# 10XGenomics/scan-rs

Hardware: NVIDIA B200
Metric: normalize+PCA cells/s, 1.3Mx33.5k, k=10 (higher is better)
Workload: dtype f64

## Files before the change

### scan_rs_b200/csrc/gather.cu

```cuda
#include <cub/cub.cuh>

#include <algorithm>
#include <numeric>

#include "common.cuh"
#include "map.cuh"

#define FULLMASK 0xffffffffu
#define GA_THREADS 1024
#define GA_STAGE_STRIDE 176u
#define GA_NONE 0xFFFFFFFFu
#define GA_TILE 20u

#define GA_ST_KEYS 16u
#define GA_ST_XS 48u
#define GA_ST_L1 112u

template <int MODE, int TAIL>
__global__ void __launch_bounds__(GA_THREADS, 1)
k_gather(const uint2 *__restrict__ ent, const GUnit *__restrict__ units, const u32 *__restrict__ item_first, u32 n_units, u32 n_items,
         u32 *__restrict__ tickets, u32 ticket_base, u32 rows, u64 n_cells, MapDev mp, const double *__restrict__ B, u32 ldb, u32 col0, u32 wt, u32 w,
         const u32 *__restrict__ slot_gene, double *__restrict__ out, u32 ldo, long long *__restrict__ cycles) {
    __shared__ u32 s_item;
    __shared__ long long s_t0;
    if (cycles && threadIdx.x == 0) s_t0 = clock64();
    extern __shared__ __align__(16) unsigned char smem_raw[];
    double *XA = reinterpret_cast<double *>(smem_raw);
    double *XB = XA + (size_t)(rows + 1) * 16;
    double *par = XB + (TAIL ? (size_t)(rows + 1) * 4 : 0);
    double *par2 = par + rows;
    LogEnt *ltab = reinterpret_cast<LogEnt *>(par2 + rows);
    unsigned char *stage_all = reinterpret_cast<unsigned char *>(ltab + 128);

    const int lane = threadIdx.x & 31, wib = threadIdx.x >> 5, nw = blockDim.x >> 5;
    const int grp = lane >> 3, lig = lane & 7;
    const u32 xa_sa = (u32)__cvta_generic_to_shared(XA) + (u32)lig * 16u;
    const u32 xb_sa = (u32)__cvta_generic_to_shared(XB) + (u32)(lig & 3) * 8u;
    const u32 stage_grp = (u32)__cvta_generic_to_shared(stage_all) + (u32)(wib * 4 + grp) * GA_STAGE_STRIDE;
    const u32 zero_off16 = rows * 8u;
    const u32 cA = 2u * lig, cB = 16u + (lig & 3);
    const bool ok0 = cA < wt && col0 + cA < w, ok1 = cA + 1 < wt && col0 + cA + 1 < w;
    const bool okb = TAIL && cB < wt && col0 + cB < w;
    const u32 wt_even = (wt + 1) & ~1u;
    const bool logchain = mp.kind == 1;
    constexpr bool TS = MODE >= 1, DEFER = MODE == 2;
    double *const oA = out + col0 + cA;
    const long long tdelta = (long long)cB - (long long)cA;
    const u32 ok0m = ok0, ok1m = ok1, okbm = okb;
    const u64 ldo64 = (u64)ldo;

    for (int i = threadIdx.x; i < 128; i += blockDim.x) ltab[i] = sb_log_table[i];

    u32 staged = GA_NONE;
    u32 first_item = GA_NONE;

    for (;;) {
    __syncthreads();
    if (threadIdx.x == 0) s_item = atomicAdd(tickets, 1u) - ticket_base;
    __syncthreads();
    const u32 item = s_item;
    if (item >= n_items) break;
    if (first_item == GA_NONE) first_item = item;
    const u32 u_begin = item_first[item], u_end = min(n_units, item_first[item + 1]);
    for (u32 ui = u_begin; ui < u_end; ui++) {
        const GUnit un = units[ui];
        if (un.panel != staged) {
            __syncthreads();
            constexpr u32 PAIRS = TAIL ? 10 : 8;
            for (u32 i = threadIdx.x; i < (rows + 1) * PAIRS; i += blockDim.x) {
                const u32 r = i / PAIRS, j2 = (i - r * PAIRS) * 2, col = col0 + j2;
                double2 val = make_double2(0.0, 0.0);
                if (r < rows && j2 < wt_even && col < w) {
                    if (MODE == 0) {
                        const u64 cell = (u64)un.panel * rows + r;
                        if (cell < n_cells) {
                            val = *reinterpret_cast<const double2 *>(B + cell * (size_t)ldb + col);
                            if (logchain) {
                                const double l1 = mp.l1[cell];
                                val.x *= l1;
                                val.y *= l1;
                            }
                        }
                    } else {
                        const u32 g = slot_gene[(size_t)un.panel * rows + r];
                        if (g != GA_NONE) {
                            val = *reinterpret_cast<const double2 *>(B + (size_t)g * ldb + col);
                            if (logchain && mp.row) {
                                const double rs = mp.row[g];
                                val.x *= rs;
                                val.y *= rs;
                            }
                        }
                    }
                }
                if (j2 < 16) *reinterpret_cast<double2 *>(XA + (size_t)r * 16 + j2) = val;
                else *reinterpret_cast<double2 *>(XB + (size_t)r * 4 + (j2 - 16)) = val;
            }
            for (u32 r = threadIdx.x; r < rows; r += blockDim.x) {
                double pv = 0.0, pv2 = 0.0;
                if (MODE == 0) {
                    const u64 cell = (u64)un.panel * rows + r;
                    if (cell < n_cells) {
                        pv = mp.col[cell];
                        if (logchain) pv2 = mp.inv_l1[cell];
                    }
                } else if (!logchain) {
                    const u32 g = slot_gene[(size_t)un.panel * rows + r];
                    if (g != GA_NONE) pv = mp.row[g];
                }
                par[r] = pv;
                par2[r] = pv2;
            }
            staged = un.panel;
            __syncthreads();
        }
        u64 span = (un.end - un.begin + nw - 1) / nw;
        span = (span + 31) & ~(u64)31;
        const u64 wb = min(un.end, un.begin + (u64)wib * span), we = min(un.end, wb + span);
        const u64 qspan = span >> 2;
        const u64 gb = min(we, wb + (u64)grp * qspan), ge = min(we, gb + qspan);
        const u32 nchunks = (u32)((min(we, wb + qspan) - wb + 7) >> 3);

        u32 cur = GA_NONE, carry = GA_NONE;
        double curL1 = 0.0;
        double a0 = 0.0, a1 = 0.0, bt = 0.0;

        auto flush = [&]() {
            if (cur == GA_NONE) return;
            if (TS && !DEFER) {
                a0 *= curL1;
                a1 *= curL1;
                bt *= curL1;
            }
            double *o = oA + (u64)cur * ldo64;
            asm volatile("{ .reg .pred p; setp.ne.u32 p, %2, 0; @p red.global.add.f64 [%0], %1; }" ::"l"(o), "d"(a0), "r"(ok0m) : "memory");
            asm volatile("{ .reg .pred p; setp.ne.u32 p, %2, 0; @p red.global.add.f64 [%0 + 8], %1; }" ::"l"(o), "d"(a1), "r"(ok1m) : "memory");
            if (TAIL) asm volatile("{ .reg .pred p; setp.ne.u32 p, %2, 0; @p red.global.add.f64 [%0], %1; }" ::"l"(o + tdelta), "d"(bt), "r"(okbm) : "memory");
            a0 = 0.0;
            a1 = 0.0;
            bt = 0.0;
        };

        uint2 znext = (gb + lig < ge) ? __ldcs(ent + gb + lig) : make_uint2(GA_NONE, 0u);
        for (u32 ch = 0; ch < nchunks; ch++) {
            const uint2 z = znext;
            const u64 kn = gb + (u64)(ch + 1) * 8 + lig;
            znext = (kn < ge) ? __ldcs(ent + kn) : make_uint2(GA_NONE, 0u);
            const bool valid = z.x != GA_NONE;
            const u32 key = z.x & SB_GENE_MASK, local = z.x >> SB_GENE_BITS;
            const bool general = valid && (!logchain || z.y != 1u);
            double x = 0.0;
            if (general) {
                if (MODE == 0) {
                    if (logchain) x = map_log_part(mp.log_base, par[local], z.y, ltab) * par2[local];
                    else x = map_full(mp, z.y, key, par[local], false, ltab);
                } else {
                    const double cp = mp.col[key];
                    if (logchain) x = map_log_part(mp.log_base, cp, z.y, ltab) * mp.inv_l1[key];
                    else x = mp.kind == 2 ? map_binom_dev((double)z.y, cp, par[local]) : map_binom_pearson((double)z.y, cp, par[local]);
                }
            }
            u32 prev = __shfl_up_sync(FULLMASK, key, 1, 8);
            if (lig == 0) prev = carry;
            const bool head = valid && key != prev;
            double l1v = 0.0;
            if (TS && !DEFER && head) l1v = logchain ? mp.l1[key] : 1.0;
            carry = __shfl_sync(FULLMASK, key, 7, 8);
            const u32 myh = (__ballot_sync(FULLMASK, head) >> (8 * grp)) & 0xFFu;
            const u32 myg = (__ballot_sync(FULLMASK, general) >> (8 * grp)) & 0xFFu;
            __syncwarp();
            asm volatile("st.shared.u16 [%0], %1;" ::"r"(stage_grp + (u32)lig * 2u), "h"((unsigned short)(valid ? local * 8u : zero_off16)) : "memory");
            asm volatile("st.shared.u32 [%0], %1;" ::"r"(stage_grp + GA_ST_KEYS + (u32)lig * 4u), "r"(key) : "memory");
            if (general) asm volatile("st.shared.f64 [%0], %1;" ::"r"(stage_grp + GA_ST_XS + (u32)lig * 8u), "d"(x) : "memory");
            if (TS && !DEFER && head) asm volatile("st.shared.f64 [%0], %1;" ::"r"(stage_grp + GA_ST_L1 + (u32)lig * 8u), "d"(l1v) : "memory");
            __syncwarp();
            u32 ov[4];
            asm volatile("ld.shared.v4.u32 {%0, %1, %2, %3}, [%4];" : "=r"(ov[0]), "=r"(ov[1]), "=r"(ov[2]), "=r"(ov[3]) : "r"(stage_grp));
#pragma unroll
            for (int s = 0; s < 8; s += 2) {
                const u32 off0 = (ov[s >> 1] & 0xFFFFu) << 4, off1 = (ov[s >> 1] >> 16) << 4;
                double tl = 0.0;
                if (TAIL) {
                    const u32 toff = (lig < 4 ? off0 : off1) >> 2;
                    asm volatile("ld.shared.f64 %0, [%1];" : "=d"(tl) : "r"(xb_sa + toff));
                }
                double x0, x1, m0 = 1.0, m1 = 1.0;
                asm volatile("{ .reg .pred p; setp.ne.u32 p, %1, 0; @p ld.shared.f64 %0, [%2]; }"
                             : "+d"(m0) : "r"(myg & (1u << s)), "r"(stage_grp + GA_ST_XS + (u32)s * 8u));
                asm volatile("{ .reg .pred p; setp.ne.u32 p, %1, 0; @p ld.shared.f64 %0, [%2]; }"
                             : "+d"(m1) : "r"(myg & (2u << s)), "r"(stage_grp + GA_ST_XS + (u32)(s + 1) * 8u));
                if (myh & (1u << s)) {
                    flush();
                    asm volatile("ld.shared.u32 %0, [%1];" : "=r"(cur) : "r"(stage_grp + GA_ST_KEYS + (u32)s * 4u));
                    if (TS && !DEFER) asm volatile("ld.shared.f64 %0, [%1];" : "=d"(curL1) : "r"(stage_grp + GA_ST_L1 + (u32)s * 8u));
                }
                asm volatile("ld.shared.v2.f64 {%0, %1}, [%2];" : "=d"(x0), "=d"(x1) : "r"(xa_sa + off0));
                a0 = fma(m0, x0, a0);
                a1 = fma(m0, x1, a1);
                if (TAIL && lig < 4) bt = fma(m0, tl, bt);
                if (myh & (2u << s)) {
                    flush();
                    asm volatile("ld.shared.u32 %0, [%1];" : "=r"(cur) : "r"(stage_grp + GA_ST_KEYS + (u32)(s + 1) * 4u));
                    if (TS && !DEFER) asm volatile("ld.shared.f64 %0, [%1];" : "=d"(curL1) : "r"(stage_grp + GA_ST_L1 + (u32)(s + 1) * 8u));
                }
                asm volatile("ld.shared.v2.f64 {%0, %1}, [%2];" : "=d"(x0), "=d"(x1) : "r"(xa_sa + off1));
                a0 = fma(m1, x0, a0);
                a1 = fma(m1, x1, a1);
                if (TAIL && lig >= 4) bt = fma(m1, tl, bt);
            }
        }
        flush();
    }
    }
    if (cycles && threadIdx.x == 0 && first_item != GA_NONE) {
        u32 smid;
        asm volatile("mov.u32 %0, %%smid;" : "=r"(smid));
        cycles[first_item] = clock64() - s_t0;
        cycles[gridDim.x + first_item] = (long long)smid;
    }
}

__global__ void k_t_init(double *__restrict__ out, u64 n, u32 w, u32 ldo, const double *__restrict__ uy, const double *__restrict__ v) {
    const u64 total = n * w;
    for (u64 i = (u64)blockIdx.x * blockDim.x + threadIdx.x; i < total; i += (u64)gridDim.x * blockDim.x) {
        const u64 c = i / w;
        const u32 j = (u32)(i - c * w);
        out[c * ldo + j] = uy ? (v ? v[c] : 1.0) * uy[j] : 0.0;
    }
}

int gather_t_init(sb_ctx *ctx, double *out, u64 n, u32 w, u32 ldo, const double *uy, const double *v) {
    if (n == 0 || w == 0) return SB_OK;
    u64 blocks = std::min<u64>((n * w + 255) / 256, (u64)ctx->sm_count * 16);
    k_t_init<<<(unsigned)blocks, 256, 0, ctx->stream>>>(out, n, w, ldo, uy, v);
    count_launch(ctx);
    return SB_OK;
}

static size_t gather_smem(u32 rows, bool tail) {
    return (size_t)(rows + 1) * (tail ? 20 : 16) * 8 + (size_t)rows * 16 + 128 * sizeof(LogEnt) + (size_t)(GA_THREADS / 32) * 4 * GA_STAGE_STRIDE;
}

int gather_run_tile(sb_ctx *ctx, const GatherLayout &L, int mode, const MapDev &mp, u64 n_cells, const double *B, u32 ldb, u32 w, u32 col0, double *out,
                    u32 ldo, long long *cycles) {
    if (!L.ready) return sb_fail(SB_ERR_UNSUPPORTED, "gather_run: layout not built");
    if (L.nnz == 0 || L.n_units == 0 || w == 0 || col0 >= w) return SB_OK;
    const u32 n_items = L.n_items ? L.n_items : L.grid;
    if (!L.tickets.p) {
        SB_TRY(L.tickets.alloc(1));
        SB_CUDA(cudaMemsetAsync(L.tickets.p, 0, sizeof(u32), ctx->stream));
        L.ticket_base = 0;
    }
    if (L.ticket_base > 0x7F000000u) {
        SB_CUDA(cudaMemsetAsync(L.tickets.p, 0, sizeof(u32), ctx->stream));
        L.ticket_base = 0;
    }
    const u32 wt = std::min(GA_TILE, w - col0);
    const bool tail = wt > 16;
    const size_t smem = gather_smem(L.rows, tail);
    cudaError_t e;
#define GA_LAUNCH(M, T)                                                                                                                        \
    e = cudaFuncSetAttribute(k_gather<M, T>, cudaFuncAttributeMaxDynamicSharedMemorySize, (int)smem);                                          \
    if (e == cudaSuccess)                                                                                                                      \
        k_gather<M, T><<<L.grid, GA_THREADS, smem, ctx->stream>>>(L.ent, L.units.p, L.cta_first.p, L.n_units, n_items, L.tickets.p, L.ticket_base, \
                                                                  L.rows, n_cells, mp, B, ldb, col0, wt, w, L.slot_gene.p, out, ldo, cycles);
    if (mode == 0) {
        if (tail) { GA_LAUNCH(0, 1) } else { GA_LAUNCH(0, 0) }
    } else if (mode == 1) {
        if (tail) { GA_LAUNCH(1, 1) } else { GA_LAUNCH(1, 0) }
    } else {
        if (tail) { GA_LAUNCH(2, 1) } else { GA_LAUNCH(2, 0) }
    }
#undef GA_LAUNCH
    if (e != cudaSuccess) return sb_fail(SB_ERR_CUDA, "gather_run: %zu B of shared memory: %s", smem, cudaGetErrorString(e));
    L.ticket_base += n_items + L.grid;
    count_launch(ctx);
    SB_CUDA(cudaGetLastError());
    return SB_OK;
}

int gather_run(sb_ctx *ctx, const GatherLayout &L, int mode, const MapDev &mp, u64 n_cells, const double *B, u32 ldb, u32 w, double *out, u32 ldo,
               long long *cycles) {
    for (u32 col0 = 0; col0 < w; col0 += GA_TILE) SB_TRY(gather_run_tile(ctx, L, mode, mp, n_cells, B, ldb, w, col0, out, ldo, col0 == 0 ? cycles : nullptr));
    return SB_OK;
}

int gather_build_n(sb_mat *mt, GatherLayout &L, const uint2 *gm, const u64 *gm_base_dev, u64 nnz) {
    sb_ctx *ctx = mt->ctx;
    L.ready = false;
    L.rows = (mt->pc + 1) & ~1u;
    if (L.rows != mt->pc) return sb_fail(SB_ERR_UNSUPPORTED, "gather_build_n: odd panel size");
    L.npanels = mt->np;
    L.ent = gm;
    L.nnz = nnz;
    std::vector<u64> base((size_t)mt->np + 1, 0);
    if (mt->np) SB_CUDA(cudaMemcpyAsync(base.data(), gm_base_dev, base.size() * sizeof(u64), cudaMemcpyDeviceToHost, ctx->stream));
    SB_CUDA(cudaStreamSynchronize(ctx->stream));
    const u32 G = (u32)ctx->sm_count;
    std::vector<GUnit> units;
    std::vector<u32> first;
    gather_units_n(base, nnz, G, units, first);
    L.n_units = (u32)units.size();
    L.grid = G;
    SB_TRY(L.units.alloc(units.size()));
    SB_TRY(L.cta_first.alloc(first.size()));
    if (!units.empty()) SB_CUDA(cudaMemcpyAsync(L.units.p, units.data(), units.size() * sizeof(GUnit), cudaMemcpyHostToDevice, ctx->stream));
    SB_CUDA(cudaMemcpyAsync(L.cta_first.p, first.data(), first.size() * sizeof(u32), cudaMemcpyHostToDevice, ctx->stream));
    SB_CUDA(cudaStreamSynchronize(ctx->stream));
    L.ready = true;
    return SB_OK;
}

__global__ void k_ent_gene_hist(const uint2 *__restrict__ ent, u64 nnz, u32 *__restrict__ hist) {
    for (u64 i = (u64)blockIdx.x * blockDim.x + threadIdx.x; i < nnz; i += (u64)gridDim.x * blockDim.x) atomicAdd(&hist[ent[i].x], 1u);
}

__global__ void k_make_tkeys(const u64 *__restrict__ ptr, const uint2 *__restrict__ ent, u64 nc, u64 c0, const u32 *__restrict__ slot_of_gene,
                             u32 rows, u32 npanels, u32 *__restrict__ keys, u64 *__restrict__ payload) {
    u64 warp = ((u64)blockIdx.x * blockDim.x + threadIdx.x) >> 5;
    u64 nwarps = ((u64)gridDim.x * blockDim.x) >> 5;
    int lane = threadIdx.x & 31;
    for (u64 v = warp; v < nc; v += nwarps) {
        const u64 s = ptr[v], e = ptr[v + 1];
        const u32 blk = (u32)(v / GA_TBLOCK);
        const u32 cell = (u32)(c0 + v);
        for (u64 k = s + lane; k < e; k += 32) {
            const uint2 z = ent[k];
            const u32 slot = slot_of_gene[z.x];
            const u32 p = slot / rows, sl = slot - p * rows;
            keys[k] = blk * npanels + p;
            payload[k] = ((u64)z.y << 32) | (u64)(cell | (sl << SB_GENE_BITS));
        }
    }
}

__global__ void k_unpack_u64(const u64 *__restrict__ payload, uint2 *__restrict__ out, u64 nnz) {
    for (u64 i = (u64)blockIdx.x * blockDim.x + threadIdx.x; i < nnz; i += (u64)gridDim.x * blockDim.x) {
        const u64 p = payload[i];
        out[i] = make_uint2((u32)p, (u32)(p >> 32));
    }
}

__global__ void k_key_first(const u32 *__restrict__ keys, const u64 *__restrict__ payload, u64 nnz, u64 *__restrict__ first,
                            unsigned long long *__restrict__ runs) {
    const int lane = threadIdx.x & 31;
    const u64 total = (nnz + 31) & ~(u64)31;
    for (u64 i = (u64)blockIdx.x * blockDim.x + threadIdx.x; i < total; i += (u64)gridDim.x * blockDim.x) {
        const bool valid = i < nnz;
        const u32 key = valid ? keys[i] : 0xFFFFFFFFu;
        bool head = false;
        if (valid) {
            const bool newkey = i == 0 || keys[i - 1] != key;
            if (newkey) first[key] = i;
            head = newkey || ((u32)payload[i - 1] & SB_GENE_MASK) != ((u32)payload[i] & SB_GENE_MASK);
        }
        const u32 key0 = __shfl_sync(FULLMASK, key, 0);
        const unsigned hm = __ballot_sync(FULLMASK, head);
        if (__all_sync(FULLMASK, !valid || key == key0)) {
            if (lane == 0 && hm) atomicAdd(&runs[key0], (unsigned long long)__popc(hm));
        } else if (head) {
            atomicAdd(&runs[key], 1ull);
        }
    }
}

static inline int ga_grid(u64 items, int threads, sb_ctx *ctx, int per_sm = 16) {
    u64 blocks = (items + threads - 1) / threads, cap = (u64)ctx->sm_count * per_sm;
    return (int)std::max<u64>(1, std::min(blocks, cap));
}

int gather_assign_slots(sb_mat *mt, const uint2 *ent, u64 nnz) {
    sb_ctx *ctx = mt->ctx;
    GatherLayout &L = mt->gt;
    L.ready = false;
    const u32 m = mt->m;
    u32 rows = std::min<u32>(SB_MAX_PANEL_CELLS, (m + 1) & ~1u);
    if (rows < 2) rows = 2;
    L.rows = rows;
    L.npanels = (m + rows - 1) / rows;
    if (L.npanels == 0) L.npanels = 1;
    DevBuf<u32> hist;
    SB_TRY(hist.alloc((size_t)m + 1));
    SB_CUDA(cudaMemsetAsync(hist.p, 0, ((size_t)m + 1) * sizeof(u32), ctx->stream));
    if (nnz) {
        k_ent_gene_hist<<<ga_grid(nnz, 256, ctx), 256, 0, ctx->stream>>>(ent, nnz, hist.p);
        count_launch(ctx);
    }
    std::vector<u32> h((size_t)m + 1);
    SB_CUDA(cudaMemcpyAsync(h.data(), hist.p, h.size() * sizeof(u32), cudaMemcpyDeviceToHost, ctx->stream));
    SB_CUDA(cudaStreamSynchronize(ctx->stream));
    std::vector<u32> order(m);
    std::iota(order.begin(), order.end(), 0u);
    std::stable_sort(order.begin(), order.end(), [&](u32 a, u32 b) { return h[a] > h[b]; });
    std::vector<u32> slot_of(m ? m : 1, 0), slot_gene((size_t)L.npanels * rows, GA_NONE);
    for (u32 r = 0; r < m; r++) {
        slot_of[order[r]] = r;
        slot_gene[r] = order[r];
    }
    SB_TRY(mt->slot_of_gene.alloc(slot_of.size()));
    SB_TRY(L.slot_gene.alloc(slot_gene.size()));
    SB_CUDA(cudaMemcpyAsync(mt->slot_of_gene.p, slot_of.data(), slot_of.size() * sizeof(u32), cudaMemcpyHostToDevice, ctx->stream));
    SB_CUDA(cudaMemcpyAsync(L.slot_gene.p, slot_gene.data(), slot_gene.size() * sizeof(u32), cudaMemcpyHostToDevice, ctx->stream));
    SB_CUDA(cudaStreamSynchronize(ctx->stream));
    return SB_OK;
}

int gather_build_t_range(sb_mat *mt, u64 c0, u64 nc, const u64 *ptr_local, const uint2 *ent, u64 nnz, DevBuf<uint2> &out, std::vector<u64> &seg_len,
                         std::vector<u64> &seg_runs) {
    sb_ctx *ctx = mt->ctx;
    GatherLayout &L = mt->gt;
    const u64 nblk = (nc + GA_TBLOCK - 1) / GA_TBLOCK;
    const u64 nkeys = nblk * L.npanels;
    seg_len.assign(nkeys, 0);
    seg_runs.assign(nkeys, 0);
    SB_TRY(out.alloc(nnz));
    if (nnz == 0 || nc == 0) return SB_OK;
    if (nkeys > 0x7FFFFFFFull) return sb_fail(SB_ERR_UNSUPPORTED, "gather: block x panel key exceeds 31 bits");
    DevBuf<u32> keys, keys2;
    DevBuf<u64> payload, payload2, first, runs;
    SB_TRY(keys.alloc(nnz));
    SB_TRY(keys2.alloc(nnz));
    SB_TRY(payload.alloc(nnz));
    SB_TRY(payload2.alloc(nnz));
    SB_TRY(first.alloc(nkeys));
    SB_TRY(runs.alloc(nkeys));
    k_make_tkeys<<<ga_grid(nc * 32, 256, ctx), 256, 0, ctx->stream>>>(ptr_local, ent, nc, c0, mt->slot_of_gene.p, L.rows, L.npanels, keys.p, payload.p);
    count_launch(ctx);
    int end_bit = 1;
    while (end_bit < 32 && ((nkeys - 1) >> end_bit)) end_bit++;
    cub::DoubleBuffer<u32> dk(keys.p, keys2.p);
    cub::DoubleBuffer<u64> dv(payload.p, payload2.p);
    size_t tmp_bytes = 0;
    SB_CUDA(cub::DeviceRadixSort::SortPairs(nullptr, tmp_bytes, dk, dv, (unsigned long long)nnz, 0, end_bit, ctx->stream));
    DevBuf<char> tmp;
    SB_TRY(tmp.alloc(tmp_bytes));
    SB_CUDA(cub::DeviceRadixSort::SortPairs(tmp.p, tmp_bytes, dk, dv, (unsigned long long)nnz, 0, end_bit, ctx->stream));
    count_launch(ctx, false);
    SB_CUDA(cudaMemsetAsync(first.p, 0xFF, nkeys * sizeof(u64), ctx->stream));
    SB_CUDA(cudaMemsetAsync(runs.p, 0, nkeys * sizeof(u64), ctx->stream));
    k_key_first<<<ga_grid(nnz, 256, ctx), 256, 0, ctx->stream>>>(dk.Current(), dv.Current(), nnz, first.p, (unsigned long long *)runs.p);
    k_unpack_u64<<<ga_grid(nnz, 256, ctx), 256, 0, ctx->stream>>>(dv.Current(), out.p, nnz);
    count_launch(ctx); count_launch(ctx);
    std::vector<u64> h(nkeys);
    SB_CUDA(cudaMemcpyAsync(h.data(), first.p, nkeys * sizeof(u64), cudaMemcpyDeviceToHost, ctx->stream));
    SB_CUDA(cudaMemcpyAsync(seg_runs.data(), runs.p, nkeys * sizeof(u64), cudaMemcpyDeviceToHost, ctx->stream));
    SB_CUDA(cudaStreamSynchronize(ctx->stream));
    u64 next = nnz;
    for (u64 k = nkeys; k-- > 0;) {
        if (h[k] == ~0ull) h[k] = next;
        seg_len[k] = next - h[k];
        next = h[k];
    }
    return SB_OK;
}

#define GA_FLUSH_COST 5.0
int gather_finish_t(sb_mat *mt, const std::vector<u64> &seg_len, const std::vector<u64> &seg_runs) {
    sb_ctx *ctx = mt->ctx;
    GatherLayout &L = mt->gt;
    u64 total_nnz = 0;
    for (u64 x : seg_len) total_nnz += x;
    L.nnz = total_nnz;
    std::vector<GUnit> units;
    std::vector<u32> first;
    mt->t_seg_len = seg_len;
    mt->t_seg_runs = seg_runs;
    mt->t_calibrated = 0;
    mt->t_rate.clear();
    const u32 per_cta = (u32)std::max(1, ctx->gather_items_per_cta);
    gather_units_t(seg_len, seg_runs, L.npanels, (u32)ctx->sm_count * per_cta, ctx->gather_flush_cost, units, first, ctx->gather_seg_cost);
    mt->t_units_host = units;
    mt->t_first_host = first;
    L.n_items = (u32)first.size() - 1;
    L.grid = std::min<u32>(L.n_items, (u32)ctx->sm_count);
    L.n_units = (u32)units.size();
    SB_TRY(L.units.alloc(units.size()));
    SB_TRY(L.cta_first.alloc(first.size()));
    if (!units.empty()) SB_CUDA(cudaMemcpyAsync(L.units.p, units.data(), units.size() * sizeof(GUnit), cudaMemcpyHostToDevice, ctx->stream));
    SB_CUDA(cudaMemcpyAsync(L.cta_first.p, first.data(), first.size() * sizeof(u32), cudaMemcpyHostToDevice, ctx->stream));
    SB_CUDA(cudaStreamSynchronize(ctx->stream));
    L.ent = L.ent_own.p;
    L.ready = true;
    return SB_OK;
}

int gather_build_t(sb_mat *mt, const u64 *ptr, const uint2 *ent, u64 nnz) {
    if (mt->n > SB_GENE_MASK) {
        mt->gt.ready = false;
        return SB_OK;
    }
    SB_TRY(gather_assign_slots(mt, ent, nnz));
    std::vector<u64> seg, runs;
    SB_TRY(gather_build_t_range(mt, 0, mt->n, ptr, ent, nnz, mt->gt.ent_own, seg, runs));
    return gather_finish_t(mt, seg, runs);
}

int gather_recalibrate_t(sb_mat *mt, const long long *cycles_dev) {
    sb_ctx *ctx = mt->ctx;
    GatherLayout &L = mt->gt;
    mt->t_calibrated++;
    if (!L.ready || L.n_items != L.grid || mt->t_units_host.empty() || L.npanels == 0) return SB_OK;
    const u32 G = L.grid, np = L.npanels;
    std::vector<long long> cyc(2 * (size_t)G, 0);
    SB_CUDA(cudaMemcpyAsync(cyc.data(), cycles_dev, 2 * (size_t)G * sizeof(long long), cudaMemcpyDeviceToHost, ctx->stream));
    SB_CUDA(cudaStreamSynchronize(ctx->stream));
    const std::vector<u64> &seg_len = mt->t_seg_len, &seg_runs = mt->t_seg_runs;
    std::vector<u64> seg_pos(seg_len.size() + 1, 0);
    for (size_t k = 0; k < seg_len.size(); k++) seg_pos[k + 1] = seg_pos[k] + seg_len[k];
    std::vector<double> cta_cost(G, 0.0), pan_cost(np, 0.0), pan_time(np, 0.0);
    struct PanelShare { u32 panel; double cost, wgt; };
    std::vector<std::vector<PanelShare>> by_panel(G);
    for (u32 b = 0; b < G; b++) {
        for (u32 ui = mt->t_first_host[b]; ui < mt->t_first_host[b + 1]; ui++) {
            const GUnit &u = mt->t_units_host[ui];
            const size_t k = (size_t)(std::upper_bound(seg_pos.begin(), seg_pos.end(), u.begin) - seg_pos.begin()) - 1;
            if (k >= seg_len.size() || seg_len[k] == 0) continue;
            const double frac = (double)(u.end - u.begin) / (double)seg_len[k];
            const double c = frac * ((double)seg_len[k] + ctx->gather_flush_cost * (double)seg_runs[k] + ctx->gather_seg_cost);
            const double wgt = c * (mt->t_rate.size() == np ? mt->t_rate[u.panel] : 1.0);
            cta_cost[b] += wgt;
            if (by_panel[b].empty() || by_panel[b].back().panel != u.panel) by_panel[b].push_back({u.panel, 0.0, 0.0});
            by_panel[b].back().cost += c;
            by_panel[b].back().wgt += wgt;
        }
    }
    for (u32 b = 0; b < G; b++) {
        if (cta_cost[b] <= 0.0 || cyc[b] <= 0) continue;
        for (auto &pc : by_panel[b]) {
            pan_cost[pc.panel] += pc.cost;
            pan_time[pc.panel] += (double)cyc[b] * pc.wgt / cta_cost[b];
        }
    }
    double tot_c = 0.0, tot_t = 0.0;
    for (u32 p = 0; p < np; p++) {
        tot_c += pan_cost[p];
        tot_t += pan_time[p];
    }
    if (const char *dump = getenv("SCANB200_GATHER_DUMP")) {
        if (FILE *f = fopen(dump, "a")) {
            fprintf(f, "# round %d\n", mt->t_calibrated);
            for (u32 b = 0; b < G; b++)
                fprintf(f, "%u %lld %lld %.6g %u %zu\n", b, cyc[G + b], cyc[b], cta_cost[b], by_panel[b].empty() ? 0u : by_panel[b].front().panel, by_panel[b].size());
            fclose(f);
        }
    }
    if (!(tot_c > 0.0) || !(tot_t > 0.0)) return SB_OK;
    const double mean_rate = tot_t / tot_c;
    std::vector<double> rate(np, 1.0);
    for (u32 p = 0; p < np; p++)
        if (pan_cost[p] > 0.0) rate[p] = std::min(4.0, std::max(0.25, (pan_time[p] / pan_cost[p]) / mean_rate));
    std::vector<GUnit> units;
    std::vector<u32> first;
    gather_units_t(seg_len, seg_runs, np, G, ctx->gather_flush_cost, units, first, ctx->gather_seg_cost, &rate);
    if ((u32)first.size() - 1 != G) return SB_OK;
    SB_TRY(L.units.alloc(units.size()));
    SB_TRY(L.cta_first.alloc(first.size()));
    if (!units.empty()) SB_CUDA(cudaMemcpyAsync(L.units.p, units.data(), units.size() * sizeof(GUnit), cudaMemcpyHostToDevice, ctx->stream));
    SB_CUDA(cudaMemcpyAsync(L.cta_first.p, first.data(), first.size() * sizeof(u32), cudaMemcpyHostToDevice, ctx->stream));
    SB_CUDA(cudaStreamSynchronize(ctx->stream));
    L.n_units = (u32)units.size();
    mt->t_units_host.swap(units);
    mt->t_first_host.swap(first);
    mt->t_rate = rate;
    if (TraceScope::on()) {
        double lo = 1e300, hi = 0.0;
        for (u32 b = 0; b < G; b++)
            if (cyc[b] > 0) { lo = std::min(lo, (double)cyc[b]); hi = std::max(hi, (double)cyc[b]); }
        fprintf(stderr, "[scanb200] gather T recalibrated: CTA cycles %.3g .. %.3g (mean rate %.3g per cost unit)\n", lo, hi, mean_rate);
    }
    return SB_OK;
}
```

Measured before the change: 17.66 million.

## Interleave XA smem layout, specialize full tiles, drop general-mask ballot

Permutes the shared XA panel so each lane accumulates columns lig and lig+8, which changes the output atomics to stride-64-byte pairs. The tail accumulator now runs on all lanes against separate per-pair tail loads. A compile-time FULL variant issues unpredicated red.global.add when the tile is full. The per-chunk ballot for general entries is removed by storing 1.0 for non-general x, the first segment key is preloaded so flush skips its null check, and the code grows through template duplication.

Result: faster. 18.35 million (median of 6 runs) (+3.9%).

```diff
diff --git a/scan_rs_b200/csrc/gather.cu b/scan_rs_b200/csrc/gather.cu
--- a/scan_rs_b200/csrc/gather.cu
+++ b/scan_rs_b200/csrc/gather.cu
@@ -2,6 +2,7 @@
 
 #include <algorithm>
 #include <numeric>
+#include <type_traits>
 
 #include "common.cuh"
 #include "map.cuh"
@@ -15,6 +16,7 @@
 #define GA_ST_KEYS 16u
 #define GA_ST_XS 48u
 #define GA_ST_L1 112u
+#define XA_SLOT(c) ((((c) & 7u) << 1) | ((c) >> 3))
 
 template <int MODE, int TAIL>
 __global__ void __launch_bounds__(GA_THREADS, 1)
@@ -38,15 +40,16 @@
     const u32 xb_sa = (u32)__cvta_generic_to_shared(XB) + (u32)(lig & 3) * 8u;
     const u32 stage_grp = (u32)__cvta_generic_to_shared(stage_all) + (u32)(wib * 4 + grp) * GA_STAGE_STRIDE;
     const u32 zero_off16 = rows * 8u;
-    const u32 cA = 2u * lig, cB = 16u + (lig & 3);
-    const bool ok0 = cA < wt && col0 + cA < w, ok1 = cA + 1 < wt && col0 + cA + 1 < w;
-    const bool okb = TAIL && cB < wt && col0 + cB < w;
+    const u32 cA = lig, cB = 16u + (lig & 3);
+    const bool ok0 = cA < wt && col0 + cA < w, ok1 = cA + 8 < wt && col0 + cA + 8 < w;
+    const bool okb = TAIL && lig < 4 && cB < wt && col0 + cB < w;
     const u32 wt_even = (wt + 1) & ~1u;
     const bool logchain = mp.kind == 1;
     constexpr bool TS = MODE >= 1, DEFER = MODE == 2;
     double *const oA = out + col0 + cA;
     const long long tdelta = (long long)cB - (long long)cA;
     const u32 ok0m = ok0, ok1m = ok1, okbm = okb;
+    const bool full = TAIL ? wt == GA_TILE : wt == 16u;
     const u64 ldo64 = (u64)ldo;
 
     for (int i = threadIdx.x; i < 128; i += blockDim.x) ltab[i] = sb_log_table[i];
@@ -93,7 +96,10 @@
                         }
                     }
                 }
-                if (j2 < 16) *reinterpret_cast<double2 *>(XA + (size_t)r * 16 + j2) = val;
+                if (j2 < 16) {
+                    XA[(size_t)r * 16 + XA_SLOT(j2)] = val.x;
+                    XA[(size_t)r * 16 + XA_SLOT(j2 + 1)] = val.y;
+                }
                 else *reinterpret_cast<double2 *>(XB + (size_t)r * 4 + (j2 - 16)) = val;
             }
             for (u32 r = threadIdx.x; r < rows; r += blockDim.x) {
@@ -121,95 +127,103 @@
         const u64 gb = min(we, wb + (u64)grp * qspan), ge = min(we, gb + qspan);
         const u32 nchunks = (u32)((min(we, wb + qspan) - wb + 7) >> 3);
 
-        u32 cur = GA_NONE, carry = GA_NONE;
-        double curL1 = 0.0;
-        double a0 = 0.0, a1 = 0.0, bt = 0.0;
-
-        auto flush = [&]() {
-            if (cur == GA_NONE) return;
-            if (TS && !DEFER) {
-                a0 *= curL1;
-                a1 *= curL1;
-                bt *= curL1;
+        auto walk = [&](auto full_t) {
+            constexpr bool FULL = decltype(full_t)::value;
+            uint2 znext = (gb + lig < ge) ? __ldcs(ent + gb + lig) : make_uint2(GA_NONE, 0u);
+
+            const u32 z0 = __shfl_sync(FULLMASK, znext.x, 0, 8);
+            u32 cur = z0 == GA_NONE ? GA_NONE : (z0 & SB_GENE_MASK), carry = cur;
+            double curL1 = 0.0;
+            if (TS && !DEFER && cur != GA_NONE) curL1 = logchain ? mp.l1[cur] : 1.0;
+            double a0 = 0.0, a1 = 0.0, bt = 0.0;
+
+            auto flush = [&]() {
+                if (TS && !DEFER) {
+                    a0 *= curL1;
+                    a1 *= curL1;
+                    bt *= curL1;
+                }
+                double *o = oA + (u64)cur * ldo64;
+                if (FULL) {
+                    asm volatile("red.global.add.f64 [%0], %1;" ::"l"(o), "d"(a0) : "memory");
+                    asm volatile("red.global.add.f64 [%0 + 64], %1;" ::"l"(o), "d"(a1) : "memory");
+                    if (TAIL && lig < 4) asm volatile("red.global.add.f64 [%0], %1;" ::"l"(o + tdelta), "d"(bt) : "memory");
+                } else {
+                    asm volatile("{ .reg .pred p; setp.ne.u32 p, %2, 0; @p red.global.add.f64 [%0], %1; }" ::"l"(o), "d"(a0), "r"(ok0m) : "memory");
+                    asm volatile("{ .reg .pred p; setp.ne.u32 p, %2, 0; @p red.global.add.f64 [%0 + 64], %1; }" ::"l"(o), "d"(a1), "r"(ok1m) : "memory");
+                    if (TAIL) asm volatile("{ .reg .pred p; setp.ne.u32 p, %2, 0; @p red.global.add.f64 [%0], %1; }" ::"l"(o + tdelta), "d"(bt), "r"(okbm) : "memory");
+                }
+                a0 = 0.0;
+                a1 = 0.0;
+                bt = 0.0;
+            };
+            for (u32 ch = 0; ch < nchunks; ch++) {
+                const uint2 z = znext;
+                const u64 kn = gb + (u64)(ch + 1) * 8 + lig;
+                znext = (kn < ge) ? __ldcs(ent + kn) : make_uint2(GA_NONE, 0u);
+                const bool valid = z.x != GA_NONE;
+                const u32 key = z.x & SB_GENE_MASK, local = z.x >> SB_GENE_BITS;
+                const bool general = valid && (!logchain || z.y != 1u);
+                double x = 0.0;
+                if (general) {
+                    if (MODE == 0) {
+                        if (logchain) x = map_log_part(mp.log_base, par[local], z.y, ltab) * par2[local];
+                        else x = map_full(mp, z.y, key, par[local], false, ltab);
+                    } else {
+                        const double cp = mp.col[key];
+                        if (logchain) x = map_log_part(mp.log_base, cp, z.y, ltab) * mp.inv_l1[key];
+                        else x = mp.kind == 2 ? map_binom_dev((double)z.y, cp, par[local]) : map_binom_pearson((double)z.y, cp, par[local]);
+                    }
+                }
+                u32 prev = __shfl_up_sync(FULLMASK, key, 1, 8);
+                if (lig == 0) prev = carry;
+                const bool head = valid && key != prev;
+                double l1v = 0.0;
+                if (TS && !DEFER && head) l1v = logchain ? mp.l1[key] : 1.0;
+                carry = __shfl_sync(FULLMASK, key, 7, 8);
+                const u32 myh = (__ballot_sync(FULLMASK, head) >> (8 * grp)) & 0xFFu;
+                __syncwarp();
+                asm volatile("st.shared.u16 [%0], %1;" ::"r"(stage_grp + (u32)lig * 2u), "h"((unsigned short)(valid ? local * 8u : zero_off16)) : "memory");
+                asm volatile("st.shared.u32 [%0], %1;" ::"r"(stage_grp + GA_ST_KEYS + (u32)lig * 4u), "r"(key) : "memory");
+                asm volatile("st.shared.f64 [%0], %1;" ::"r"(stage_grp + GA_ST_XS + (u32)lig * 8u), "d"(general ? x : 1.0) : "memory");
+                if (TS && !DEFER && head) asm volatile("st.shared.f64 [%0], %1;" ::"r"(stage_grp + GA_ST_L1 + (u32)lig * 8u), "d"(l1v) : "memory");
+                __syncwarp();
+                u32 ov[4];
+                asm volatile("ld.shared.v4.u32 {%0, %1, %2, %3}, [%4];" : "=r"(ov[0]), "=r"(ov[1]), "=r"(ov[2]), "=r"(ov[3]) : "r"(stage_grp));
+    #pragma unroll
+                for (int s = 0; s < 8; s += 2) {
+                    const u32 off0 = (ov[s >> 1] & 0xFFFFu) << 4, off1 = (ov[s >> 1] >> 16) << 4;
+                    double tl0 = 0.0, tl1 = 0.0;
+                    if (TAIL) {
+                        asm volatile("ld.shared.f64 %0, [%1];" : "=d"(tl0) : "r"(xb_sa + (off0 >> 2)));
+                        asm volatile("ld.shared.f64 %0, [%1];" : "=d"(tl1) : "r"(xb_sa + (off1 >> 2)));
+                    }
+                    double x0, x1, m0, m1;
+                    asm volatile("ld.shared.v2.f64 {%0, %1}, [%2];" : "=d"(m0), "=d"(m1) : "r"(stage_grp + GA_ST_XS + (u32)s * 8u));
+                    if (myh & (1u << s)) {
+                        flush();
+                        asm volatile("ld.shared.u32 %0, [%1];" : "=r"(cur) : "r"(stage_grp + GA_ST_KEYS + (u32)s * 4u));
+                        if (TS && !DEFER) asm volatile("ld.shared.f64 %0, [%1];" : "=d"(curL1) : "r"(stage_grp + GA_ST_L1 + (u32)s * 8u));
+                    }
+                    asm volatile("ld.shared.v2.f64 {%0, %1}, [%2];" : "=d"(x0), "=d"(x1) : "r"(xa_sa + off0));
+                    a0 = fma(m0, x0, a0);
+                    a1 = fma(m0, x1, a1);
+                    if (TAIL) bt = fma(m0, tl0, bt);
+                    if (myh & (2u << s)) {
+                        flush();
+                        asm volatile("ld.shared.u32 %0, [%1];" : "=r"(cur) : "r"(stage_grp + GA_ST_KEYS + (u32)(s + 1) * 4u));
+                        if (TS && !DEFER) asm volatile("ld.shared.f64 %0, [%1];" : "=d"(curL1) : "r"(stage_grp + GA_ST_L1 + (u32)(s + 1) * 8u));
+                    }
+                    asm volatile("ld.shared.v2.f64 {%0, %1}, [%2];" : "=d"(x0), "=d"(x1) : "r"(xa_sa + off1));
+                    a0 = fma(m1, x0, a0);
+                    a1 = fma(m1, x1, a1);
+                    if (TAIL) bt = fma(m1, tl1, bt);
+                }
             }
-            double *o = oA + (u64)cur * ldo64;
-            asm volatile("{ .reg .pred p; setp.ne.u32 p, %2, 0; @p red.global.add.f64 [%0], %1; }" ::"l"(o), "d"(a0), "r"(ok0m) : "memory");
-            asm volatile("{ .reg .pred p; setp.ne.u32 p, %2, 0; @p red.global.add.f64 [%0 + 8], %1; }" ::"l"(o), "d"(a1), "r"(ok1m) : "memory");
-            if (TAIL) asm volatile("{ .reg .pred p; setp.ne.u32 p, %2, 0; @p red.global.add.f64 [%0], %1; }" ::"l"(o + tdelta), "d"(bt), "r"(okbm) : "memory");
-            a0 = 0.0;
-            a1 = 0.0;
-            bt = 0.0;
+            if (cur != GA_NONE) flush();
         };
-
-        uint2 znext = (gb + lig < ge) ? __ldcs(ent + gb + lig) : make_uint2(GA_NONE, 0u);
-        for (u32 ch = 0; ch < nchunks; ch++) {
-            const uint2 z = znext;
-            const u64 kn = gb + (u64)(ch + 1) * 8 + lig;
-            znext = (kn < ge) ? __ldcs(ent + kn) : make_uint2(GA_NONE, 0u);
-            const bool valid = z.x != GA_NONE;
-            const u32 key = z.x & SB_GENE_MASK, local = z.x >> SB_GENE_BITS;
-            const bool general = valid && (!logchain || z.y != 1u);
-            double x = 0.0;
-            if (general) {
-                if (MODE == 0) {
-                    if (logchain) x = map_log_part(mp.log_base, par[local], z.y, ltab) * par2[local];
-                    else x = map_full(mp, z.y, key, par[local], false, ltab);
-                } else {
-                    const double cp = mp.col[key];
-                    if (logchain) x = map_log_part(mp.log_base, cp, z.y, ltab) * mp.inv_l1[key];
-                    else x = mp.kind == 2 ? map_binom_dev((double)z.y, cp, par[local]) : map_binom_pearson((double)z.y, cp, par[local]);
-                }
-            }
-            u32 prev = __shfl_up_sync(FULLMASK, key, 1, 8);
-            if (lig == 0) prev = carry;
-            const bool head = valid && key != prev;
-            double l1v = 0.0;
-            if (TS && !DEFER && head) l1v = logchain ? mp.l1[key] : 1.0;
-            carry = __shfl_sync(FULLMASK, key, 7, 8);
-            const u32 myh = (__ballot_sync(FULLMASK, head) >> (8 * grp)) & 0xFFu;
-            const u32 myg = (__ballot_sync(FULLMASK, general) >> (8 * grp)) & 0xFFu;
-            __syncwarp();
-            asm volatile("st.shared.u16 [%0], %1;" ::"r"(stage_grp + (u32)lig * 2u), "h"((unsigned short)(valid ? local * 8u : zero_off16)) : "memory");
-            asm volatile("st.shared.u32 [%0], %1;" ::"r"(stage_grp + GA_ST_KEYS + (u32)lig * 4u), "r"(key) : "memory");
-            if (general) asm volatile("st.shared.f64 [%0], %1;" ::"r"(stage_grp + GA_ST_XS + (u32)lig * 8u), "d"(x) : "memory");
-            if (TS && !DEFER && head) asm volatile("st.shared.f64 [%0], %1;" ::"r"(stage_grp + GA_ST_L1 + (u32)lig * 8u), "d"(l1v) : "memory");
-            __syncwarp();
-            u32 ov[4];
-            asm volatile("ld.shared.v4.u32 {%0, %1, %2, %3}, [%4];" : "=r"(ov[0]), "=r"(ov[1]), "=r"(ov[2]), "=r"(ov[3]) : "r"(stage_grp));
-#pragma unroll
-            for (int s = 0; s < 8; s += 2) {
-                const u32 off0 = (ov[s >> 1] & 0xFFFFu) << 4, off1 = (ov[s >> 1] >> 16) << 4;
-                double tl = 0.0;
-                if (TAIL) {
-                    const u32 toff = (lig < 4 ? off0 : off1) >> 2;
-                    asm volatile("ld.shared.f64 %0, [%1];" : "=d"(tl) : "r"(xb_sa + toff));
-                }
-                double x0, x1, m0 = 1.0, m1 = 1.0;
-                asm volatile("{ .reg .pred p; setp.ne.u32 p, %1, 0; @p ld.shared.f64 %0, [%2]; }"
-                             : "+d"(m0) : "r"(myg & (1u << s)), "r"(stage_grp + GA_ST_XS + (u32)s * 8u));
-                asm volatile("{ .reg .pred p; setp.ne.u32 p, %1, 0; @p ld.shared.f64 %0, [%2]; }"
-                             : "+d"(m1) : "r"(myg & (2u << s)), "r"(stage_grp + GA_ST_XS + (u32)(s + 1) * 8u));
-                if (myh & (1u << s)) {
-                    flush();
-                    asm volatile("ld.shared.u32 %0, [%1];" : "=r"(cur) : "r"(stage_grp + GA_ST_KEYS + (u32)s * 4u));
-                    if (TS && !DEFER) asm volatile("ld.shared.f64 %0, [%1];" : "=d"(curL1) : "r"(stage_grp + GA_ST_L1 + (u32)s * 8u));
-                }
-                asm volatile("ld.shared.v2.f64 {%0, %1}, [%2];" : "=d"(x0), "=d"(x1) : "r"(xa_sa + off0));
-                a0 = fma(m0, x0, a0);
-                a1 = fma(m0, x1, a1);
-                if (TAIL && lig < 4) bt = fma(m0, tl, bt);
-                if (myh & (2u << s)) {
-                    flush();
-                    asm volatile("ld.shared.u32 %0, [%1];" : "=r"(cur) : "r"(stage_grp + GA_ST_KEYS + (u32)(s + 1) * 4u));
-                    if (TS && !DEFER) asm volatile("ld.shared.f64 %0, [%1];" : "=d"(curL1) : "r"(stage_grp + GA_ST_L1 + (u32)(s + 1) * 8u));
-                }
-                asm volatile("ld.shared.v2.f64 {%0, %1}, [%2];" : "=d"(x0), "=d"(x1) : "r"(xa_sa + off1));
-                a0 = fma(m1, x0, a0);
-                a1 = fma(m1, x1, a1);
-                if (TAIL && lig >= 4) bt = fma(m1, tl, bt);
-            }
-        }
-        flush();
+        if (full) walk(std::true_type{});
+        else walk(std::false_type{});
     }
     }
     if (cycles && threadIdx.x == 0 && first_item != GA_NONE) {
```
